# NCKempke/PIPS-IPMpp

Hardware: AMD Instinct MI355X
Metric: KKT factor+solve per IPM iter/sec, N-block arrowhead LP (higher is better)
Workload: dtype f64; 1 GPU; 64 blocks x 10000 vars (5000 eq rows, rho=0.001), Schur dim 2000, 64 blocks/GPU [BASELINE configs[1]]; deterministic=False, family=random, root=dense LDL^T, sparse_head=multifrontal (k_front), solves_per_unit=4, collective=none, nnzL_per_gpu=649118456

## Files before the change

### include/pips_hip.h

```cpp
#ifndef PIPS_HIP_H
#define PIPS_HIP_H
#include <stddef.h>
#include <stdint.h>

#ifdef __cplusplus
extern "C" {
#endif

const char* pips_hip_last_error(void);
long long pips_hip_host_wait_count(void);
int pips_hip_host_wait_sites(char* buf, int cap);
int pips_hip_device_count(void);

int pips_hip_ldl_create(void** handle, int n, const int* krow, const int* jcol, int device, int flags);
int pips_hip_ldl_set_inertia_hint(void* handle, int n_primal);
int pips_hip_ldl_set_pivot_rule(void* handle, double thr_rel, double repl_rel);
int pips_hip_ldl_set_refinement(void* handle, int max_steps, double tol);
int pips_hip_ldl_set_refinement_backward_error(void* handle, int max_steps, double tol);
int pips_hip_ldl_set_deterministic(void* handle, int on);
int pips_hip_ldl_analyze(void* handle);
int pips_hip_ldl_factor(void* handle, const double* vals_host);
int pips_hip_ldl_solve(void* handle, int nrhs, double* rhs_inout_host, int ld);
int pips_hip_ldl_inertia(void* handle, int* pos, int* neg, int* zero);
int pips_hip_ldl_set_border(void* handle, int S, const int* Bt_rowptr, const int* Bt_colidx);
int pips_hip_ldl_factor_schur(void* handle, const double* K_vals_host, const double* Bt_vals_host, double* SC_host, int ldSC);
int pips_hip_ldl_solve_dev(void* handle, int nrhs, double* rhs_inout_dev, long long ld);
int pips_hip_ldl_solve_sparse(void* handle, int nrhs, double* rhs_inout_host, int ld, const int* col_sparsity);
int pips_hip_ldl_factor_schur_batch(void* const* handles, int n, const double* const* K_vals_host, const double* const* Bt_vals_host,
                                    double* SC_host, int ldSC);
int pips_hip_ldl_solve_batch(void* const* handles, int n, double* const* rhs_inout_host);
int pips_hip_ldl_solve_batch_dev(void* const* handles, int n, double* x_dev);
int pips_hip_ldl_inertia_batch(void* const* handles, int n, int* pos, int* neg, int* zero);
int pips_hip_ldl_info(void* handle, int64_t* what, int n_what);
int pips_hip_ldl_get_perm(void* handle, int* perm);
void pips_hip_ldl_destroy(void* handle);

int pips_hip_dense_ldl_create(void** handle, int n, int n_primal, int device);
int pips_hip_dense_ldl_set_pivoting(void* handle, int mode);
int pips_root_plan_build(int ntc, int workers, int qmin, int urgent, int chain_slots, int* out, long long cap, long long* n_tasks,
                         long long* n_chain_tasks, double* makespan_us);
int pips_hip_dense_ldl_set_distributed(void* handle, void* comm, int rank, int n_ranks);
int pips_hip_dense_ldl_factor(void* handle, const double* A_host, int lda);
int pips_hip_dense_ldl_factor_dev(void* handle, const double* A_dev, int lda);
int pips_hip_dense_ldl_solve(void* handle, int nrhs, double* rhs_inout_host, int ld);
int pips_hip_dense_ldl_solve_dev(void* handle, double* rhs_inout_dev);
int pips_hip_dense_ldl_inertia(void* handle, int* pos, int* neg, int* zero);
void pips_hip_dense_ldl_destroy(void* handle);

int pips_hip_batch_create(void** handle, int n_blocks, int S, int device, void* stream);
int pips_hip_batch_set_block(void* handle, int b, int n, int n_primal, const int* K_rowptr, const int* K_colidx,
                             const int* Bt_rowptr, const int* Bt_colidx, const double* Bt_val);
int pips_hip_batch_set_options(void* handle, int force_n_head, int refine_steps, double thr_rel, double repl_rel);
int pips_hip_batch_set_schur_mode(void* handle, int mode);
int pips_hip_batch_get_schur_mode(void* handle, int* mode);
int pips_hip_batch_set_deterministic(void* handle, int on);
int pips_hip_batch_add_regularization(void* handle, double primal, double dual);
int pips_hip_batch_set_refinement(void* handle, int max_steps, double tol);
int pips_hip_batch_set_refinement_backward_error(void* handle, int max_steps, double tol);
double pips_hip_batch_last_refinement_measure(void* handle);
int pips_hip_batch_last_refinement_steps(void* handle);
int pips_hip_batch_analyze(void* handle, int n_threads);
int pips_hip_batch_set_values(void* handle, int b, const double* K_val_host);
int pips_hip_batch_set_diagonals_dev(void* handle, const double* diag_dev);
// ... 169 lines not shown
```

### pips-ipmpp_amd/csrc/engine.hip

```cpp
#include <hip/hip_runtime.h>

#include <algorithm>
#include <cstdlib>
#include <cstring>
#include <map>
#include <memory>
#include <mutex>
#include <thread>
#include <vector>

#include "common.h"
#include "kernels.hip.h"
#include "rootkernel.hip.h"
#include "tailkernel.hip.h"
#include "pips_hip.h"

namespace pips {

static thread_local std::string g_last_error;
void set_last_error(const std::string& msg) { g_last_error = msg; }
std::atomic<long long> g_host_waits{0};
struct WaitSite { std::atomic<const char*> file{nullptr}; std::atomic<int> line{0}; std::atomic<long long> n{0}; };
static WaitSite g_wait_sites[128];
void note_host_wait(const char* file, int line) {
// ... 28 lines not shown
   HIP_TRY(hipMalloc((void**)dptr, bytes));
   if (!h.empty()) HIP_TRY(hipMemcpy(*dptr, h.data(), h.size() * sizeof(T), hipMemcpyHostToDevice));
   return PIPS_OK;
}

static int env_int(const char* name, int dflt) {
   const char* v = getenv(name);
   return v ? atoi(v) : dflt;
}

static inline int grid_for(long long n, int block, int cap = 4096) {
   long long g = (n + block - 1) / block;
   if (g < 1) g = 1;
   if (g > cap) g = cap;
   return (int)g;
}

struct TaskList { long long off = 0; int cnt = 0; };

struct TailPlan {
   int ntc_max = 0;
   std::vector<TaskList> upd, upd_diag, diag, trsm, fwd, bwd, trail, trail_next;
   TaskList schur;
   TileTask* d_tasks = nullptr;
   std::vector<TileTask> h_tasks;

   int build(const std::vector<BlkDesc>& blks, int panel = 0, bool lookahead = false, bool split_diag = false,
             const std::vector<const std::vector<int>*>* first = nullptr, bool diag_ahead = false, int pair2 = 1) {
      std::vector<TileTask> all;
      ntc_max = 0;
      for (auto& b : blks) ntc_max = std::max(ntc_max, b.ntc);
      upd.assign(ntc_max, {});
      upd_diag.assign(ntc_max, {});
      diag.assign(ntc_max, {});
      trsm.assign(ntc_max, {});
      fwd.assign(ntc_max, {});
      bwd.assign(ntc_max, {});
      trail.assign(ntc_max, {});
      trail_next.assign(ntc_max, {});
      const int nblk = (int)blks.size();
      auto begin = [&](TaskList& l) { l.off = (long long)all.size(); };
      auto end = [&](TaskList& l) { l.cnt = (int)((long long)all.size() - l.off); };
      for (int j = 0; j < ntc_max; ++j) {
         const int p0 = panel > 0 ? j / panel * panel : 0;
         auto fst = [&](int b, int t) { return first ? (*(*first)[b])[t] : 0; };
         begin(upd_diag[j]);
         if (j > p0 && split_diag)
            for (int b = 0; b < nblk; ++b)
               if (blks[b].ntc > j) {
                  const int k0 = std::max(p0, fst(b, j));
                  if (k0 < j) all.push_back({b, j, j, (diag_ahead ? std::max(k0, j - 1) : k0) | (j << 16)});
               }
         end(upd_diag[j]);
         begin(upd[j]);
         const int P = (pair2 > 1 && panel == 0 && split_diag && diag_ahead) ? pair2 : 1;
         const int g = j / P * P, q = j - g;
         if (j > p0 && split_diag && diag_ahead)
            for (int b = 0; b < nblk; ++b)
               if (blks[b].ntc > j + 1) {
                  const int k0 = std::max(p0, fst(b, j + 1)), lo = q > 0 ? std::max(k0, g) : k0;
                  if (lo < j) all.push_back({b, j + 1, j + 1, lo | (j << 16)});
               }
         if (P > 1 && q == 0 && j > p0)
            for (int b = 0; b < nblk; ++b)
               for (int d = j + 2; d <= j + P && d < blks[b].ntc; ++d) {
                  const int k0 = std::max(p0, fst(b, d));
                  if (k0 < j) all.push_back({b, d, d, k0 | (j << 16)});
               }
         if (j > p0)
            for (int b = 0; b < nblk; ++b)
               if (blks[b].ntc > j)
                  for (int ti = split_diag ? j + 1 : j; ti < blks[b].ntr; ++ti) {
                     if (j >= fst(b, ti)) {
                        const int k0 = std::max({p0, fst(b, ti), fst(b, j)}), lo = q > 0 ? std::max(k0, g) : k0;
                        if (lo < j) all.push_back({b, ti, j, lo | (j << 16)});
                     }
                     if (P > 1 && q == 0)
                        for (int c = j + 1; c < j + P && c < blks[b].ntc && c < ti; ++c)
                           if (c >= fst(b, ti)) {
                              const int k0 = std::max({p0, fst(b, ti), fst(b, c)});
                              if (k0 < j) all.push_back({b, ti, c, k0 | (j << 16)});
                           }
                  }
         end(upd[j]);
         begin(diag[j]);
         for (int b = 0; b < nblk; ++b)
            if (blks[b].ntc > j) all.push_back({b, j, j, 0});
         end(diag[j]);
         begin(trsm[j]);
         for (int b = 0; b < nblk; ++b)
            if (blks[b].ntc > j)
               for (int ti = j + 1; ti < blks[b].ntr; ++ti)
                  if (j >= fst(b, ti)) all.push_back({b, ti, j, 0});
         end(trsm[j]);
         begin(fwd[j]);
         for (int b = 0; b < nblk; ++b)
            if (blks[b].ntc > j)
               for (int ti = j; ti < blks[b].ntc; ++ti)
                  if (ti == j || (j >= 1 && j - 1 >= fst(b, ti))) all.push_back({b, ti, j, 0});
         end(fwd[j]);
         begin(bwd[j]);
         for (int b = 0; b < nblk; ++b)
            if (blks[b].ntc > j)
               for (int tj = 0; tj <= j; ++tj)
                  if (tj == j || (j + 1 < blks[b].ntc && tj >= fst(b, j + 1))) all.push_back({b, tj, j, 0});
         end(bwd[j]);
         if (panel > 0 && (j + 1) % panel == 0) {
            begin(trail_next[j]);
            if (lookahead)
               for (int b = 0; b < nblk; ++b)
                  if (j + 1 < blks[b].ntc)
                     for (int ti = j + 1; ti < blks[b].ntr; ++ti) all.push_back({b, ti, j + 1, p0 | ((j + 1) << 16)});
            end(trail_next[j]);
            begin(trail[j]);
            for (int b = 0; b < nblk; ++b)
               for (int tj = j + (lookahead ? 2 : 1); tj < blks[b].ntc; ++tj)
                  for (int ti = tj; ti < blks[b].ntr; ++ti) all.push_back({b, ti, tj, p0 | ((j + 1) << 16)});
            end(trail[j]);
         }
      }
      begin(schur);
      for (int b = 0; b < nblk; ++b)
         if (blks[b].ntc > 0 && blks[b].nb > 0) {
            const int nt = blks[b].nb_pad / TILE;
            for (int ti = 0; ti < nt; ++ti)
               for (int tj = 0; tj <= ti; ++tj) all.push_back({b, ti, tj, 0});
         }
      end(schur);
      h_tasks = all;
      return dev_upload(&d_tasks, all, nullptr);
   }
   void release() {
      if (d_tasks) (void)hipFree(d_tasks);
      d_tasks = nullptr;
   }
};

struct SweepRt {
   TileTask* d_tasks = nullptr;
   int n_tasks = 0;
   int* d_ints = nullptr;
   long long n_flags = 0;
   long long* d_flag_off = nullptr;
   int* d_tfirst = nullptr;
   long long* d_tfirst_off = nullptr;
   int epoch = 0;
   bool enabled = false;
   long long poll_limit = SWEEP_POLL_LIMIT;
   int take_error(const char* who) {
      if (!d_ints) return PIPS_OK;
      int w = 0;
      HIP_TRY(hipMemcpy(&w, d_ints + 2 * SWEEP_NRHS_MAX, sizeof(int), hipMemcpyDeviceToHost));
      if (!w) return PIPS_OK;
// ... 197 lines not shown
   double* d_uarena = nullptr;
   const std::vector<TaskList>* sc_groups = nullptr;
   const TileTask* d_sc_tasks = nullptr;
   const std::vector<hipEvent_t>* ev_sc = nullptr;
   int* d_ctr_pool = nullptr;
   int* ctr_cursor = nullptr;
   const std::vector<TaskList>* det_rounds = nullptr;
   const TileTask* d_det_tasks = nullptr;
   double* d_gbuf = nullptr;
   long long gstride = 0;
   const int* d_blk_group = nullptr;
   int n_groups = 0, first_slot = 0;
   long long sc_len = 0;
   bool det_defer_reduce = false;
   bool det_reduce_later = false;
   SweepRt* sweep = nullptr;
   bool bunch_kaufman = false;
   int *d_pert_cnt = nullptr, *d_pert_list = nullptr;
   const double* bk_orig = nullptr;
   int bk_orig_ld = 0, bk_orig_rowmajor = 0;
   const int* d_bk_perm = nullptr;
   int bk_isolate = 0;
   const TailSingle* single = nullptr;
};
constexpr int GEMM_CTR_SLOTS = 4096;
constexpr int GEMM_BAL_MIN_TASKS = 1024;

static void reduce_det_groups(const TailCtx& c, double* SC, int ldSC) {
   const int S_ = ldSC;
   if (c.det_defer_reduce) {
   } else if (c.d_sctab)
      hipLaunchKernelGGL(k_reduce_groups, dim3((unsigned)std::max(1LL, std::min(1024LL, (c.sc_len + 255) / 256)), 1), dim3(256), 0, c.stream, SC, 0, (int)c.sc_len,
                         c.d_gbuf, c.gstride, c.n_groups, c.first_slot);
   else
      hipLaunchKernelGGL(k_reduce_groups, dim3(std::max(1, std::min(64, (S_ + 255) / 256)), S_), dim3(256), 0, c.stream, SC, ldSC, S_, c.d_gbuf,
                         c.gstride, c.n_groups, c.first_slot);
}

static int tail_factor(const TailCtx& c, double* SC, int ldSC) {
   const TailPlan& p = *c.plan;
   auto gemm_diag_tiles = [&](const TaskList& l, hipStream_t st) {
      hipLaunchKernelGGL(k_tile_gemm<4>, dim3((l.cnt + 7) / 8 * 8), dim3(512), 0, st, p.d_tasks + l.off, l.cnt, c.d_blks, c.d_arena,
                         c.d_dtail, c.d_winv, c.d_bmap, (double*)nullptr, 0, (const int*)nullptr, c.d_uarena);
   };
   auto gemm0 = [&](const TaskList& l, hipStream_t st) {
      if (!c.is_root && c.d_ctr_pool && l.cnt >= GEMM_BAL_MIN_TASKS && *c.ctr_cursor < GEMM_CTR_SLOTS) {
         int* ctr = c.d_ctr_pool + 8 * (*c.ctr_cursor)++;
         const int wgs = ((l.cnt + 7) / 8 * 8) / 8 * 9;
         hipLaunchKernelGGL(k_tile_gemm_bal<0>, dim3((wgs + 7) / 8 * 8), dim3(512), 0, st, p.d_tasks + l.off, l.cnt, c.d_blks, c.d_arena, c.d_dtail,
                            c.d_winv, c.d_bmap, (double*)nullptr, 0, (const int*)nullptr, c.d_uarena, ctr);
         return;
      }
      if (c.is_root)
         hipLaunchKernelGGL(k_tile_gemm<3>, dim3((l.cnt + 7) / 8 * 8), dim3(512), 0, st, p.d_tasks + l.off, l.cnt, c.d_blks, c.d_arena,
                            c.d_dtail, c.d_winv, c.d_bmap, (double*)nullptr, 0, (const int*)nullptr, c.d_uarena);
      else
         hipLaunchKernelGGL(k_tile_gemm<0>, dim3((l.cnt + 7) / 8 * 8), dim3(512), 0, st, p.d_tasks + l.off, l.cnt, c.d_blks, c.d_arena,
                            c.d_dtail, c.d_winv, c.d_bmap, (double*)nullptr, 0, (const int*)nullptr, c.d_uarena);
   };
   bool side_busy = false;
   int side_from = 0;
   auto main_writes = [&](int col) -> int {
      if (side_busy && col >= side_from) {
         HIP_TRY(hipStreamWaitEvent(c.stream, c.ev_rest, 0));
         side_busy = false;
      }
      return PIPS_OK;
   };
   int rc;
   if (c.single && c.single->n_tasks > 0) {
      const TailSingle& ts = *c.single;
      if (c.timer) c.timer->begin(c.stream, 2);
      HIP_TRY(hipMemcpyAsync(ts.d_flags, ts.d_flags_init, (size_t)ts.n_flags * sizeof(int), hipMemcpyDeviceToDevice, c.stream));
      HIP_TRY(hipMemsetAsync(ts.d_ctl, 0, 9 * sizeof(int), c.stream));
      TailLdlArgs ta = ts.args;
      ta.n_tasks = ts.n_tasks;
      const char* trace_file = getenv("PIPS_HIP_TAIL_TRACE");
      long long* d_trace = nullptr;
      const size_t n_trace = (size_t)3 * ts.n_tasks + 32 * (size_t)(p.ntc_max + 1);
      if (trace_file) {
         HIP_TRY(hipMalloc((void**)&d_trace, n_trace * sizeof(long long)));
         HIP_TRY(hipMemsetAsync(d_trace, 0, n_trace * sizeof(long long), c.stream));
         ta.trace = d_trace;
      }
      hipLaunchKernelGGL(k_tail_ldl, dim3(ts.n_blocks <= 2 ? 256 : 512), dim3(512), 0, c.stream, ta);
      if (c.timer) c.timer->end(c.stream);
      if (trace_file) {
         std::vector<long long> h(n_trace);
         std::vector<TileTask> ht((size_t)ts.n_tasks);
         HIP_TRY(hipStreamSynchronize(c.stream));
         HIP_TRY(hipMemcpy(h.data(), d_trace, h.size() * sizeof(long long), hipMemcpyDeviceToHost));
         HIP_TRY(hipMemcpy(ht.data(), ts.d_tasks, ht.size() * sizeof(TileTask), hipMemcpyDeviceToHost));
// ... 31 lines not shown
         gemm0(p.upd[j], c.stream);
         if (c.timer) c.timer->end(c.stream);
      }
      if (ahead) {
         HIP_TRY(hipStreamWaitEvent(c.stream, c.ev_rest, 0));
      } else {
         if (c.timer) c.timer->begin(c.stream, 3);
         if (c.bunch_kaufman)
            hipLaunchKernelGGL(k_tile_diag_bk, dim3(p.diag[j].cnt), dim3(256), 0, c.stream, p.d_tasks + p.diag[j].off, c.d_blks, c.d_arena, c.d_dtail,
                               c.d_winv, c.d_inertia, c.d_pert_cnt, c.d_pert_list, c.bk_orig, c.bk_orig_ld, c.bk_orig_rowmajor, c.d_bk_perm, c.bk_isolate);
         else
         hipLaunchKernelGGL(k_tile_diag, dim3(p.diag[j].cnt), dim3(256), 0, c.stream, p.d_tasks + p.diag[j].off,
                            c.d_blks, c.d_arena, c.d_dtail, c.d_winv, c.d_psign, c.d_psign_off, c.d_inertia, c.d_pref);
         if (c.timer) c.timer->end(c.stream);
      }
      if (p.trsm[j].cnt > 0) {
         if (c.timer) c.timer->begin(c.stream, 4);
         hipLaunchKernelGGL(k_tile_gemm<1>, dim3((p.trsm[j].cnt + 7) / 8 * 8), dim3(512), 0, c.stream, p.d_tasks + p.trsm[j].off, p.trsm[j].cnt,
                            c.d_blks, c.d_arena, c.d_dtail, c.d_winv, c.d_bmap, (double*)nullptr, 0, (const int*)nullptr, c.d_uarena);
         if (c.timer) c.timer->end(c.stream);
         if (c.bunch_kaufman && c.is_root && c.d_pert_cnt)
            hipLaunchKernelGGL(k_bk_growth, dim3(TILE), dim3(256), 0, c.stream, c.d_blks, c.d_arena, j, 1e8, c.d_pert_cnt, c.d_pert_list);
      }
      if (p.trail_next[j].cnt > 0 || p.trail[j].cnt > 0) {
         if ((rc = main_writes(j + 1))) return rc;
         const bool split = c.side && p.trail[j].cnt > 0;
         if (split) {
            HIP_TRY(hipEventRecord(c.ev_panel, c.stream));
            HIP_TRY(hipStreamWaitEvent(c.side, c.ev_panel, 0));
            gemm0(p.trail[j], c.side);
            HIP_TRY(hipEventRecord(c.ev_rest, c.side));
            side_busy = true;
            side_from = j + 2;
         }
         if (c.timer) c.timer->begin(c.stream, 2);
         if (p.trail_next[j].cnt > 0) gemm0(p.trail_next[j], c.stream);
         if (!split && p.trail[j].cnt > 0) gemm0(p.trail[j], c.stream);
         if (c.timer) c.timer->end(c.stream);
      }
   }
   if ((rc = main_writes(1 << 30))) return rc;
   if (SC && c.det_rounds) {
      if (c.timer) c.timer->begin(c.stream, 5);
      for (const TaskList& l : *c.det_rounds)
         if (l.cnt > 0)
            hipLaunchKernelGGL(k_tile_gemm<2>, dim3((l.cnt + 7) / 8 * 8), dim3(512), 0, c.stream, c.d_det_tasks + l.off, l.cnt, c.d_blks, c.d_arena,
                               c.d_dtail, c.d_winv, c.d_bmap, SC, ldSC, c.d_sctab, c.d_uarena, c.d_gbuf, c.gstride, c.d_blk_group);
      if (!c.det_reduce_later) reduce_det_groups(c, SC, ldSC);
      if (c.timer) c.timer->end(c.stream);
   } else if (SC && c.sc_groups && !c.d_sctab) {
      if (c.timer) c.timer->begin(c.stream, 5);
      for (size_t g = 0; g < c.sc_groups->size(); ++g) {
         const TaskList& l = (*c.sc_groups)[g];
         if (l.cnt > 0)
            hipLaunchKernelGGL(k_tile_gemm<2>, dim3((l.cnt + 7) / 8 * 8), dim3(512), 0, c.stream, c.d_sc_tasks + l.off, l.cnt, c.d_blks, c.d_arena,
                               c.d_dtail, c.d_winv, c.d_bmap, SC, ldSC, c.d_sctab, c.d_uarena);
         HIP_TRY(hipEventRecord((*c.ev_sc)[g], c.stream));
      }
      if (c.timer) c.timer->end(c.stream);
   } else if (SC && p.schur.cnt > 0 && c.d_ctr_pool && !c.d_sctab && *c.ctr_cursor < GEMM_CTR_SLOTS) {
      if (c.timer) c.timer->begin(c.stream, 5);
      const int wgs = ((p.schur.cnt + 7) / 8 * 8) / 8 * 9;
      hipLaunchKernelGGL(k_tile_gemm_bal<2>, dim3((wgs + 7) / 8 * 8), dim3(512), 0, c.stream, p.d_tasks + p.schur.off, p.schur.cnt, c.d_blks,
                         c.d_arena, c.d_dtail, c.d_winv, c.d_bmap, SC, ldSC, c.d_sctab, c.d_uarena, c.d_ctr_pool + 8 * (*c.ctr_cursor)++);
// ... 151 lines not shown
   long long *d_kdst = nullptr, *d_bdst = nullptr, *d_kdiag = nullptr, *d_kptr = nullptr, *d_psign_off = nullptr,
             *d_perm_off = nullptr, *d_rowbase = nullptr, *d_bt_xoff = nullptr;
   SnDesc* d_sns = nullptr;
   BlkDesc* d_blks = nullptr;
   int *d_lf_rows = nullptr, *d_lf_ptr = nullptr, *d_lf_src = nullptr, *d_lf_pos = nullptr;
   double* d_lf_val = nullptr;
   long long lf_rows = 0, lf_entries = 0;
   LeafDesc* d_leafdesc = nullptr;
   int* d_lb_list = nullptr;
   int n_lb = 0, nb_pad_max = 0;
   int head_wcap = HEAD_WMAX;
   int *d_rowidx = nullptr, *d_upd = nullptr, *d_sncol = nullptr, *d_bmap = nullptr, *d_perm = nullptr, *d_inertia = nullptr, *d_nprimal = nullptr;
   int *d_br_rowptr = nullptr, *d_br_sc = nullptr, *d_br_src = nullptr;
   int *d_krowptr = nullptr, *d_kcolidx = nullptr, *d_bt_rowptr = nullptr, *d_bt_colidx = nullptr, *d_bt_rowsc = nullptr;
   signed char* d_psign = nullptr;
   std::vector<int> h_inertia;
   std::vector<double> h_amax;

   ~Engine() {
      release();
      if (side) (void)hipStreamDestroy(side);
      if (ev_diag_in) (void)hipEventDestroy(ev_diag_in);
      if (ev_diag_out) (void)hipEventDestroy(ev_diag_out);
   }
   void release() {
      if (d_uarena) (void)hipFree(d_uarena);
      d_uarena = nullptr;
      for (auto ev : ev_sc) (void)hipEventDestroy(ev);
      ev_sc.clear(); sc_groups.clear(); sc_row_begin.clear();
      if (d_sc_tasks) (void)hipFree(d_sc_tasks);
      d_sc_tasks = nullptr;
      for (void* q : {(void*)d_lf_rows, (void*)d_lf_ptr, (void*)d_lf_src, (void*)d_lf_pos, (void*)d_lf_val})
         if (q) (void)hipFree(q);
      d_lf_rows = d_lf_ptr = d_lf_src = d_lf_pos = nullptr; d_lf_val = nullptr;
      for (void* q : {(void*)d_br_rowptr, (void*)d_br_sc, (void*)d_br_src})
         if (q) (void)hipFree(q);
      d_br_rowptr = d_br_sc = d_br_src = nullptr;
      if (d_leafdesc) (void)hipFree(d_leafdesc);
      d_leafdesc = nullptr;
      lf_rows = 0; lf_entries = 0;
      if (d_mfU) (void)hipFree(d_mfU);
      if (d_mfLV) (void)hipFree(d_mfLV);
      for (void* q : {(void*)d_bb_batches, (void*)d_bb_meta, (void*)d_bb_off, (void*)d_bb_pos, (void*)d_bb_round_blk, (void*)d_bb_out})
         if (q) (void)hipFree(q);
      d_bb_out = nullptr;
      d_bb_batches = nullptr; d_bb_meta = nullptr; d_bb_off = nullptr; d_bb_pos = nullptr; d_bb_round_blk = nullptr; n_bb = 0; bb_doubles = 0;
// ... 42 lines not shown
      h_mmeasure = nullptr;
      mx_cap = 0;
      hostx_cap = hostpack_cap = 0;
      d_kdst = d_bdst = d_kdiag = d_kptr = d_psign_off = d_perm_off = d_rowbase = d_bt_xoff = nullptr;
      d_sns = nullptr; d_blks = nullptr;
      d_nprimal = nullptr;
      d_spine = d_spine_off = d_schur_cols = d_schur_slot = d_sctab = nullptr;
      for (void* q : {(void*)d_kb_rec, (void*)d_kb_off, (void*)d_kb_list, (void*)d_kb_tail}) if (q) (void)hipFree(q);
      d_kb_rec = nullptr; d_kb_off = nullptr; d_kb_list = nullptr; d_kb_tail = nullptr; n_kb_tail = 0; kb_level_off.clear(); kb_level_pairs.clear(); kb_level_lds.clear();
      d_frowptr = d_fcol = d_fsrc = nullptr; d_flong = nullptr;
      d_rowidx = d_upd = d_sncol = d_bmap = d_perm = d_inertia = d_krowptr = d_kcolidx = d_bt_rowptr = d_bt_colidx = d_bt_rowsc = nullptr;
      d_psign = nullptr;
      plan.release();
      sweep.release();
      tsingle.release();
   }

   SweepRt sweep;
   TailSingle tsingle;
   bool tail_single = false;
   long long tail_scratch = 0;
   hipStream_t side = nullptr;
   hipEvent_t ev_diag_in = nullptr, ev_diag_out = nullptr;
   struct GatherList {
      long long n_targets = 0, n_slots = 0;
      long long *d_tgt = nullptr, *d_off = nullptr, *d_slots = nullptr;
      void release() {
         for (void* p : {(void*)d_tgt, (void*)d_off, (void*)d_slots})
            if (p) (void)hipFree(p);
         d_tgt = d_off = d_slots = nullptr;
         n_targets = n_slots = 0;
      }
   };
   struct SlotEntry { long long target, slot; };
   bool deterministic = false;
   bool head_slots = false;
   bool slot_solves = false;
   static constexpr long long HEAD_SLOTS_MAX = 400LL * 1000 * 1000;
   long long slots_total = 0, vslots_total = 0;
   double *d_slot_val = nullptr, *d_vslot_val = nullptr;
   int last_multi_path = 0;
   double* d_mvslot = nullptr;
   std::vector<GatherList> g_levels, gv_levels;
   GatherList g_tail, g_sc, gv_tail;
   std::vector<SlotEntry> sc_e_keep;
   std::vector<int> sc_blk_keep;
// ... 178 lines not shown
            int q = (int)(std::upper_bound(sc_row_begin.begin(), sc_row_begin.end(), first) - sc_row_begin.begin()) - 1;
            q = std::max(0, std::min(q, n_panels - 1));
            for (int tj = 0; tj <= ti; ++tj) g[q].push_back({b, ti, tj, 0});
         }
      }
      std::vector<TileTask> all;
      for (int q = 0; q < n_panels; ++q) {
         TaskList l;
         l.off = (long long)all.size(); l.cnt = (int)g[q].size();
         all.insert(all.end(), g[q].begin(), g[q].end());
         sc_groups.push_back(l);
         hipEvent_t ev;
         HIP_TRY(hipEventCreateWithFlags(&ev, hipEventDisableTiming));
         ev_sc.push_back(ev);
      }
      if (all.empty()) all.push_back({-1, 0, 0, 0});
      return dev_upload(&d_sc_tasks, all, stream);
   }
   TailCtx ctx() {
      TailCtx c{d_blks, &plan, d_arena, d_dtail, d_winv, d_psign, d_psign_off, d_bmap, d_inertia, stream,
                timer.on ? &timer : nullptr, d_pref, side, ev_diag_in, ev_diag_out, false, d_sctab, d_uarena};
      if (!sc_groups.empty()) { c.sc_groups = &sc_groups; c.d_sc_tasks = d_sc_tasks; c.ev_sc = &ev_sc; }
      c.d_ctr_pool = d_gemm_ctr; c.ctr_cursor = &gemm_ctr_cursor;
      if (deterministic && d_gbuf) {
         c.det_rounds = &det_rounds; c.d_det_tasks = d_det_tasks; c.d_gbuf = d_gbuf; c.gstride = det_gstride(); c.sc_len = sc_len; c.d_blk_group = d_blk_group;
         c.n_groups = det_n_groups; c.first_slot = det_first_slot;
         c.det_defer_reduce = det_global && defer_group_reduce;
      }
      c.sweep = &sweep;
      if (tail_single) {
         tsingle.args.blks = d_blks; tsingle.args.arena = d_arena; tsingle.args.uarena = d_uarena; tsingle.args.winv = d_winv; tsingle.args.dtail = d_dtail;
         tsingle.args.pref = d_pref; tsingle.args.psign = d_psign; tsingle.args.psign_off = d_psign_off; tsingle.args.inertia = d_inertia;
         c.single = &tsingle;
      }
      return c;
   }

   int analyze_host(int n_threads, bool with_border = true) {
      sym.assign(nblk, BlockSym());
      std::vector<int> rc(nblk, 0);
      std::vector<std::string> msgs(nblk);
      n_threads = std::max(1, std::min(n_threads, nblk));
      auto work = [&](int t) {
         for (int b = t; b < nblk; b += n_threads) {
            CsrPattern K{in[b].n, in[b].n, in[b].krow.data(), in[b].kcol.data()};
            CsrPattern B{0, in[b].n, nullptr, nullptr};
// ... 572 lines not shown
      if ((rc = dev_upload(&d_bt_rowsc, h_bt_rowsc, stream))) return rc;
      if (bt_rows_total > 0 && nnzB_total > 0 && nnzB_total < (1LL << 31)) {
         std::vector<int> rp((size_t)n_total + 1, 0);
         for (long long r = 0; r < bt_rows_total; ++r)
            for (int p = h_bt_rowptr[r]; p < h_bt_rowptr[r + 1]; ++p) ++rp[h_bt_xoff[r] + h_bt_colidx[p] + 1];
         for (long long i = 0; i < n_total; ++i) rp[i + 1] += rp[i];
         std::vector<int> sc((size_t)nnzB_total), src((size_t)nnzB_total), fill(rp.begin(), rp.end() - 1);
         for (long long r = 0; r < bt_rows_total; ++r)
            for (int p = h_bt_rowptr[r]; p < h_bt_rowptr[r + 1]; ++p) {
               const int q = fill[h_bt_xoff[r] + h_bt_colidx[p]]++;
               sc[q] = h_bt_rowsc[r]; src[q] = p;
            }
         if ((rc = dev_upload(&d_br_rowptr, rp, stream)) || (rc = dev_upload(&d_br_sc, sc, stream)) || (rc = dev_upload(&d_br_src, src, stream)))
            return rc;
      }
      {
         std::vector<int> np(nblk);
         for (int b = 0; b < nblk; ++b) np[b] = in[b].n_primal;
         if ((rc = dev_upload(&d_nprimal, np, stream))) return rc;
      }
      std::vector<const std::vector<int>*> firsts(nblk);
      for (int b = 0; b < nblk; ++b) firsts[b] = &sym[b].tile_first;
      const int pair2 = 4;
      if ((rc = plan.build(h_blks, 0, false, true, &firsts, true, pair2))) return rc;
      if ((rc = sweep.build(h_blks, &firsts))) return rc;
      if (tail_single) {
         if ((rc = tsingle.build(plan, h_blks, stream))) return rc;
         tsingle.args.poll_limit = env_int("PIPS_HIP_ROOT_POLL_LIMIT", 400000) > 0 ? (long long)env_int("PIPS_HIP_ROOT_POLL_LIMIT", 400000) * 50 : 0;
         tsingle.args.diag_blocked = env_int("PIPS_HIP_ROOT_DIAG_BARRIERS", 0) ? 0 : 1;
      }
      {
         double fwd_entries = 0.0, border_entries = 0.0;
         for (int b = 0; b < nblk; ++b) {
            const BlockSym& sb = sym[b];
            fwd_entries += 0.5 * (double)sb.m_pad * sb.m_pad;
            border_entries += (double)sb.nb_pad * sb.m_pad;
            for (const HeadSupernode& sn : sb.sn) {
               const int nbord = sn.r - sn.rb;
               fwd_entries += (double)sn.w * (sn.r - nbord) + 0.5 * sn.w * sn.w;
               border_entries += (double)sn.w * nbord;
            }
         }
         border_backward_ok = schur_mode_eff == 1 && nnzB_total > 0 && (sweep.enabled || plan.ntc_max == 0) && !deterministic && border_entries <= 3.0 * fwd_entries;
         if (const char* bb = getenv("PIPS_HIP_BORDER_BACKWARD"))
            border_backward_ok = atoi(bb) != 0 && schur_mode_eff == 1 && nnzB_total > 0 && sweep.enabled && !deterministic;
         const bool aug_paths = schur_mode_eff == 1 && nnzB_total > 0 && (sweep.enabled || plan.ntc_max == 0) && spine_total == 0 &&
                                (deterministic || !head_slots);
         aug_sweeps_ok = aug_paths && border_entries <= 3.0 * fwd_entries;
         if (const char* as = getenv("PIPS_HIP_AUG_SWEEPS")) aug_sweeps_ok = atoi(as) != 0 && aug_paths;
      }
      if (!side) {
         int prio_lo = 0, prio_hi = 0;
         HIP_TRY(hipDeviceGetStreamPriorityRange(&prio_lo, &prio_hi));
         HIP_TRY(hipStreamCreateWithPriority(&side, hipStreamNonBlocking, prio_hi));
         HIP_TRY(hipEventCreateWithFlags(&ev_diag_in, hipEventDisableTiming));
         HIP_TRY(hipEventCreateWithFlags(&ev_diag_out, hipEventDisableTiming));
      }
      h_inertia.assign(3 * nblk, 0);
      slots_total = slots_acc; vslots_total = vslots_acc;
      h_sns_keep = h_sns;
      analyzed = true;
      ++analysis_gen;
      factored = false;
      head_slots = false;
      const bool want_slots = deterministic;
      if (want_slots && slots_total + vslots_total <= HEAD_SLOTS_MAX) {
         if ((rc = build_deterministic(n_threads))) return rc;
         head_slots = true;
      } else if (deterministic)
         PIPS_FAIL(PIPS_ERR_STATE, "deterministic mode: %lld head contributions exceed the slot budget of %lld", slots_total + vslots_total, HEAD_SLOTS_MAX);
      if (deterministic && (rc = set_det_groups(0, 1))) return rc;
      return PIPS_OK;
   }

   std::vector<SnDesc> h_sns_keep;
   ScatterCtx sx_atomic() const { return ScatterCtx{0, nullptr, nullptr, nullptr, nullptr}; }
   void launch_head_level(const LevelRange& L, double* SC, int ldSC, const ScatterCtx& sx) {
      if (L.simple_cnt > 0)
         hipLaunchKernelGGL(k_head_factor_simple, dim3((L.simple_cnt + 255) / 256), dim3(256), 0, stream, d_sns, L.simple_begin,
// ... 3391 lines not shown
   }
   std::vector<int> hv(hubs, hubs + n_hubs), pv, cc;
   if (!hub_dissected_order(n, ap, ai, hv, min_size, pv, cc)) PIPS_FAIL(PIPS_ERR_STATE, "pips_symbolic_probe_hubs: no separators");
   AnalyzeOptions opt;
   apply_tuning(opt);
   opt.user_perm = pv.data();
   opt.user_colcount = cc.data();
   {
      int cut = 0;
      while (cut < n - n_hubs && cc[cut] <= ROOT_ND_MAX_COLCOUNT) ++cut;
      opt.force_n_head = cut;
   }
   CsrPattern K{n, n, krow, jcol};
   CsrPattern B{0, n, nullptr, nullptr};
   std::vector<BlockSym> sym(1);
   int rc = analyze_block(K, B, n_primal, opt, sym[0]);
   if (rc) return rc;
   if (what) sym_info(sym, what, n_what);
   if (perm) std::copy(sym[0].perm.begin(), sym[0].perm.end(), perm);
   if (colcount) std::copy(sym[0].colcount.begin(), sym[0].colcount.end(), colcount);
   return PIPS_OK;
}

}
```

### pips-ipmpp_amd/csrc/kernels.hip.h

```cpp
#pragma once
#include <hip/hip_runtime.h>
#include <stdint.h>

namespace pips {

constexpr int TILE = 128;
constexpr int KB = 16;
constexpr int LDS_PAD = 16;
constexpr int LDSW = TILE + LDS_PAD;

struct SnDesc {
   long long panel;
   long long rows;
   long long upd;
   int w, r, c0, blk;
   int n_useg, rb;
   int ld, pad_;
   long long slot;
   long long vslot;
   long long U;
   long long mf;
   long long bb;
};

// ... 1472 lines not shown
                                                         const int* __restrict__ sctab, double* __restrict__ uarena,
                                                         int* __restrict__ ctr) {
   __shared__ GemmShared sh;
   __shared__ int s_tix;
   if (threadIdx.x == 0) {
      const int per = (n_tasks + 7) >> 3;
      const int xcc = (int)(__builtin_amdgcn_s_getreg((3 << 11) | 20 ) & 7);
      int got = -1;
      for (int d = 0; d < 8 && got < 0; ++d) {
         const int x = (xcc + d) & 7;
         if (__hip_atomic_load(ctr + x, __ATOMIC_RELAXED, __HIP_MEMORY_SCOPE_AGENT) >= per) continue;
         const int t = __hip_atomic_fetch_add(ctr + x, 1, __ATOMIC_RELAXED, __HIP_MEMORY_SCOPE_AGENT);
         const int tix = x * per + t;
         if (t < per && tix < n_tasks) got = tix;
      }
      s_tix = got;
   }
   __syncthreads();
   const int tix = s_tix;
   if (tix < 0) return;
   tile_gemm_body<MODE>(tix, sh, tasks, n_tasks, blks, arena, dtail, winv, bmap, SC, ldSC, sctab, uarena);
}

__global__ void k_reduce_groups(double* __restrict__ SC, int ld, int S, const double* __restrict__ gbuf, long long gstride, int n_groups,
                                int first_slot) {
   const int c = blockIdx.y;
   for (int r = c + blockIdx.x * blockDim.x + threadIdx.x; r < S; r += gridDim.x * blockDim.x) {
      const long long off = r + (long long)c * ld;
      double p[8];
#pragma unroll
      for (int g = 0; g < 8; ++g) {
         const int lg = g - first_slot;
         p[g] = (lg >= 0 && lg < n_groups) ? gbuf[lg * gstride + off] : 0.0;
      }
      SC[off] += ((p[0] + p[1]) + (p[2] + p[3])) + ((p[4] + p[5]) + (p[6] + p[7]));
   }
}



struct DiagShared {
   double colk[2][TILE];
   double xrow[2][TILE];
   double dk[TILE];
   double prs[TILE];
   int sgn[TILE];
// ... 1720 lines not shown
```

### pips-ipmpp_amd/python/capi.py

```python
import ctypes as C
import sys
import os

import numpy as np

try:
    import torch
except Exception:
    torch = None

_HERE = os.path.dirname(os.path.abspath(__file__))
LIB_PATH = os.environ.get("PIPS_HIP_LIBRARY") or os.path.join(os.path.dirname(_HERE), "libpipship.so")


class PipsHipError(RuntimeError):
    pass


def _load():
    if not os.path.exists(LIB_PATH):
        raise PipsHipError(
            f"{LIB_PATH} is missing: build it with `python -c 'import __graft_entry__ as g; g.build()'` "
            "(hipcc --offload-arch=gfx950). The MI355X backend has no CPU fallback.")
    return C.CDLL(LIB_PATH, mode=C.RTLD_GLOBAL)


lib = _load()

_i32p = np.ctypeslib.ndpointer(dtype=np.int32, flags="C_CONTIGUOUS")
_f64p = np.ctypeslib.ndpointer(dtype=np.float64, flags="C_CONTIGUOUS")
_i64p = np.ctypeslib.ndpointer(dtype=np.int64, flags="C_CONTIGUOUS")
_vp = C.c_void_p

lib.pips_hip_last_error.restype = C.c_char_p
lib.pips_hip_device_count.restype = C.c_int
lib.pips_hip_host_wait_count.restype = C.c_longlong

SYMBOLS = [
    "pips_hip_last_error", "pips_hip_device_count",
    "pips_hip_ldl_create", "pips_hip_ldl_set_inertia_hint", "pips_hip_ldl_set_pivot_rule", "pips_hip_ldl_set_refinement", "pips_hip_ldl_set_refinement_backward_error", "pips_hip_ldl_set_deterministic",
    "pips_hip_ldl_analyze", "pips_hip_ldl_factor", "pips_hip_ldl_solve", "pips_hip_ldl_inertia", "pips_hip_ldl_info",
    "pips_hip_ldl_get_perm", "pips_hip_ldl_set_border", "pips_hip_ldl_factor_schur", "pips_hip_ldl_destroy",
    "pips_hip_ldl_solve_dev", "pips_hip_ldl_solve_sparse", "pips_hip_ldl_factor_schur_batch", "pips_hip_ldl_solve_batch", "pips_hip_ldl_solve_batch_dev",
    "pips_hip_ldl_inertia_batch",
    "pips_hip_dense_ldl_create", "pips_hip_dense_ldl_factor", "pips_hip_dense_ldl_factor_dev", "pips_hip_dense_ldl_solve",
    "pips_hip_dense_ldl_solve_dev", "pips_hip_dense_ldl_inertia", "pips_hip_dense_ldl_set_pivoting", "pips_hip_dense_ldl_set_distributed", "pips_hip_dense_ldl_destroy", "pips_root_plan_build", "pips_hip_host_wait_count", "pips_hip_host_wait_sites",
    "pips_hip_batch_create", "pips_hip_batch_set_block", "pips_hip_batch_set_options", "pips_hip_batch_set_schur_mode", "pips_hip_batch_set_deterministic", "pips_hip_batch_get_schur_mode", "pips_hip_batch_add_regularization", "pips_hip_batch_set_refinement",
    "pips_hip_batch_last_refinement_steps", "pips_hip_batch_set_refinement_backward_error",
    "pips_hip_batch_last_refinement_measure", "pips_hip_batch_analyze",
    "pips_hip_batch_set_values", "pips_hip_batch_set_diagonals_dev", "pips_hip_batch_set_diagonals", "pips_hip_batch_factor",
    "pips_hip_batch_solve_dev", "pips_hip_batch_solve", "pips_hip_batch_border_tmult_dev", "pips_hip_batch_border_mult_dev",
    "pips_hip_batch_inertia", "pips_hip_batch_info", "pips_hip_batch_sync", "pips_hip_batch_set_timing",
    "pips_hip_batch_get_timing", "pips_hip_batch_destroy",
    "pips_hip_kkt_create", "pips_hip_kkt_create_sparse", "pips_hip_kkt_get_schur_sparse", "pips_hip_kkt_sparse_root_info", "pips_hip_kkt_factorize", "pips_hip_kkt_set_root_regularization", "pips_hip_kkt_solve_compressed", "pips_hip_kkt_get_schur",
    "pips_hip_kkt_set_root_inequalities", "pips_hip_kkt_set_zdiag0_dev",
    "pips_hip_kkt_root_inertia", "pips_hip_kkt_get_timing", "pips_hip_kkt_last_ltsolve_from_factor", "pips_hip_kkt_last_solve_path", "pips_hip_kkt_set_solve_check", "pips_hip_kkt_solve_check_counts", "pips_hip_kkt_set_solve_graph", "pips_hip_kkt_set_root_stream", "pips_hip_kkt_solve_graph_stats", "pips_hip_kkt_set_root_pivoting", "pips_hip_kkt_destroy",
    "pips_hip_malloc", "pips_hip_free", "pips_hip_memcpy_h2d", "pips_hip_memcpy_d2h", "pips_hip_memset",
    "pips_hip_comm_unique_id", "pips_hip_comm_create", "pips_hip_comm_create_external", "pips_hip_comm_set_external_rsag", "pips_hip_comm_set_external_broadcast", "pips_hip_broadcast", "pips_hip_comm_has_broadcast", "pips_hip_allreduce_sum_rsag", "pips_hip_all_gather", "pips_hip_comm_size", "pips_hip_allreduce_sum", "pips_hip_comm_destroy",
    "pips_hip_vec_axpy", "pips_hip_vec_axpby", "pips_hip_vec_scale", "pips_hip_vec_copy", "pips_hip_vec_set",
    "pips_hip_vec_add_const", "pips_hip_vec_mul", "pips_hip_vec_div", "pips_hip_vec_add_product", "pips_hip_vec_add_quotient",
    "pips_hip_vec_divide_some", "pips_hip_vec_select_nonzeros", "pips_hip_vec_safe_invert", "pips_hip_vec_gondzio_projection", "pips_hip_vec_dot",
    "pips_hip_vec_one_norm", "pips_hip_vec_inf_norm", "pips_hip_vec_min", "pips_hip_vec_sumsq_scaled", "pips_hip_vec_stepbound",
    "pips_hip_vec_find_blocking", "pips_hip_vec_weighted_stepbounds", "pips_hip_vec_dot_shifted", "pips_ipm_create", "pips_ipm_create_rank", "pips_ipm_create_general", "pips_ipm_get_dims", "pips_ipm_get_iterate", "pips_ipm_get_stats2", "pips_ipm_get_schur_mode", "pips_ipm_mult", "pips_ipm_outer_solve", "pips_ipm_solve", "pips_ipm_set_gondzio", "pips_ipm_set_option", "pips_ipm_set_free_variables", "pips_ipm_get_solution", "pips_ipm_get_trace", "pips_ipm_get_stats", "pips_ipm_destroy",
    "pips_gdx_read_block", "pips_gdx_block_counts", "pips_gdx_block_vector", "pips_gdx_block_matrix", "pips_gdx_block_destroy",
    "pips_gen_row_nnz", "pips_gen_block", "pips_gen_root", "pips_gen_diagonal", "pips_kkt_leaf_assemble",
    "pips_border_assemble", "pips_symbolic_probe", "pips_symbolic_probe_hubs", "pips_map_children_to_ranks",
]


# ... 968 lines not shown
```

Baseline: 8.239 64-block work units/s (1 factorize + 4 solveCompressed).

## Defer border-row tile updates into strip kernels on a low-priority side stream

Removes border rows (ti >= ntc) from the per-column update and trsm task lists. They are processed instead in column strips of width W (default 4) by a new k_border_strip kernel. That kernel runs update, update and trsm sequentially per column inside one block, on a low-priority stream that overlaps with the main diagonal/panel chain. The goal is to shorten the critical path of the tail factorization by taking the bulk border work off the per-column launches. The cost is extra event synchronization, possible contention between streams, and fine-grained ordering inside the strip kernel that relies on threadfence and syncthreads. A host-only planning export is also added for testing.

```diff
diff --git a/include/pips_hip.h b/include/pips_hip.h
--- a/include/pips_hip.h
+++ b/include/pips_hip.h
@@ -39,6 +39,8 @@
 int pips_hip_dense_ldl_set_pivoting(void* handle, int mode);
 int pips_root_plan_build(int ntc, int workers, int qmin, int urgent, int chain_slots, int* out, long long cap, long long* n_tasks,
                          long long* n_chain_tasks, double* makespan_us);
+int pips_tail_plan_tasks(int nblk, const int* ntc, const int* ntr, const int* first, int pair2, int strips, int* out, long long cap,
+                         long long* n_rows);
 int pips_hip_dense_ldl_set_distributed(void* handle, void* comm, int rank, int n_ranks);
 int pips_hip_dense_ldl_factor(void* handle, const double* A_host, int lda);
 int pips_hip_dense_ldl_factor_dev(void* handle, const double* A_dev, int lda);
diff --git a/pips-ipmpp_amd/csrc/engine.hip b/pips-ipmpp_amd/csrc/engine.hip
--- a/pips-ipmpp_amd/csrc/engine.hip
+++ b/pips-ipmpp_amd/csrc/engine.hip
@@ -74,12 +74,16 @@
    int ntc_max = 0;
    std::vector<TaskList> upd, upd_diag, diag, trsm, fwd, bwd, trail, trail_next;
    TaskList schur;
+   int strip_w = 0;
+   std::vector<TaskList> strip;
    TileTask* d_tasks = nullptr;
    std::vector<TileTask> h_tasks;
+   bool host_only = false;
 
    int build(const std::vector<BlkDesc>& blks, int panel = 0, bool lookahead = false, bool split_diag = false,
-             const std::vector<const std::vector<int>*>* first = nullptr, bool diag_ahead = false, int pair2 = 1) {
+             const std::vector<const std::vector<int>*>* first = nullptr, bool diag_ahead = false, int pair2 = 1, int strips = 0) {
       std::vector<TileTask> all;
+      strip_w = panel == 0 ? std::max(strips, 0) : 0;
       ntc_max = 0;
       for (auto& b : blks) ntc_max = std::max(ntc_max, b.ntc);
       upd.assign(ntc_max, {});
@@ -93,9 +97,11 @@
       const int nblk = (int)blks.size();
       auto begin = [&](TaskList& l) { l.off = (long long)all.size(); };
       auto end = [&](TaskList& l) { l.cnt = (int)((long long)all.size() - l.off); };
+      auto fst = [&](int b, int t) { return first ? (*(*first)[b])[t] : 0; };
+      const int P = (pair2 > 1 && panel == 0 && split_diag && diag_ahead) ? pair2 : 1;
+      auto rows_end = [&](int b) { return strip_w > 0 ? blks[b].ntc : blks[b].ntr; };
       for (int j = 0; j < ntc_max; ++j) {
          const int p0 = panel > 0 ? j / panel * panel : 0;
-         auto fst = [&](int b, int t) { return first ? (*(*first)[b])[t] : 0; };
          begin(upd_diag[j]);
          if (j > p0 && split_diag)
             for (int b = 0; b < nblk; ++b)
@@ -105,7 +111,6 @@
                }
          end(upd_diag[j]);
          begin(upd[j]);
-         const int P = (pair2 > 1 && panel == 0 && split_diag && diag_ahead) ? pair2 : 1;
          const int g = j / P * P, q = j - g;
          if (j > p0 && split_diag && diag_ahead)
             for (int b = 0; b < nblk; ++b)
@@ -122,7 +127,7 @@
          if (j > p0)
             for (int b = 0; b < nblk; ++b)
                if (blks[b].ntc > j)
-                  for (int ti = split_diag ? j + 1 : j; ti < blks[b].ntr; ++ti) {
+                  for (int ti = split_diag ? j + 1 : j; ti < rows_end(b); ++ti) {
                      if (j >= fst(b, ti)) {
                         const int k0 = std::max({p0, fst(b, ti), fst(b, j)}), lo = q > 0 ? std::max(k0, g) : k0;
                         if (lo < j) all.push_back({b, ti, j, lo | (j << 16)});
@@ -142,7 +147,7 @@
          begin(trsm[j]);
          for (int b = 0; b < nblk; ++b)
             if (blks[b].ntc > j)
-               for (int ti = j + 1; ti < blks[b].ntr; ++ti)
+               for (int ti = j + 1; ti < rows_end(b); ++ti)
                   if (j >= fst(b, ti)) all.push_back({b, ti, j, 0});
          end(trsm[j]);
          begin(fwd[j]);
@@ -171,6 +176,28 @@
             end(trail[j]);
          }
       }
+      strip.assign(strip_w > 0 ? (ntc_max + strip_w - 1) / strip_w : 0, {});
+      for (size_t sp = 0; sp < strip.size(); ++sp) {
+         begin(strip[sp]);
+         const int c0 = (int)sp * strip_w;
+         for (int b = 0; b < nblk; ++b)
+            if (blks[b].ntc > c0)
+               for (int ti = blks[b].ntc; ti < blks[b].ntr; ++ti)
+                  for (int c = c0; c < c0 + strip_w; ++c) {
+                     TileTask u1{-1, 0, 0, 0}, u2{-1, 0, 0, 0}, tr{-1, 0, 0, 0};
+                     if (c < blks[b].ntc && c >= fst(b, ti)) {
+                        const int k0 = std::max(fst(b, ti), fst(b, c)), g = c / P * P, lo = std::max(k0, g);
+                        if (g > 0 && k0 < g) u1 = {b, ti, c, k0 | (g << 16)};
+                        if (lo < c) u2 = {b, ti, c, lo | (c << 16)};
+                        tr = {b, ti, c, 0};
+                     }
+                     all.push_back(u1);
+                     all.push_back(u2);
+                     all.push_back(tr);
+                  }
+         end(strip[sp]);
+         strip[sp].cnt /= 3 * strip_w;
+      }
       begin(schur);
       for (int b = 0; b < nblk; ++b)
          if (blks[b].ntc > 0 && blks[b].nb > 0) {
@@ -180,7 +207,7 @@
          }
       end(schur);
       h_tasks = all;
-      return dev_upload(&d_tasks, all, nullptr);
+      return host_only ? PIPS_OK : dev_upload(&d_tasks, all, nullptr);
    }
    void release() {
       if (d_tasks) (void)hipFree(d_tasks);
@@ -424,6 +451,9 @@
    const int* d_bk_perm = nullptr;
    int bk_isolate = 0;
    const TailSingle* single = nullptr;
+   hipStream_t strips = nullptr;
+   hipEvent_t ev_strip_in = nullptr;
+   hipEvent_t ev_strip_out = nullptr;
 };
 constexpr int GEMM_CTR_SLOTS = 4096;
 constexpr int GEMM_BAL_MIN_TASKS = 1024;
@@ -470,6 +500,7 @@
       return PIPS_OK;
    };
    int rc;
+   bool strips_queued = false;
    if (c.single && c.single->n_tasks > 0) {
       const TailSingle& ts = *c.single;
       if (c.timer) c.timer->begin(c.stream, 2);
@@ -547,6 +578,21 @@
          if (c.bunch_kaufman && c.is_root && c.d_pert_cnt)
             hipLaunchKernelGGL(k_bk_growth, dim3(TILE), dim3(256), 0, c.stream, c.d_blks, c.d_arena, j, 1e8, c.d_pert_cnt, c.d_pert_list);
       }
+      if (p.strip_w > 0 && ((j + 1) % p.strip_w == 0 || j + 1 == p.ntc_max)) {
+         const TaskList& l = p.strip[j / p.strip_w];
+         const hipStream_t st = c.strips ? c.strips : c.stream;
+         if (l.cnt > 0) {
+            if (st != c.stream) {
+               HIP_TRY(hipEventRecord(c.ev_strip_in, c.stream));
+               HIP_TRY(hipStreamWaitEvent(st, c.ev_strip_in, 0));
+               strips_queued = true;
+            }
+            if (c.timer) c.timer->begin(st, 2);
+            hipLaunchKernelGGL(k_border_strip, dim3((l.cnt + 7) / 8 * 8), dim3(512), 0, st, p.d_tasks + l.off, l.cnt, p.strip_w, c.d_blks,
+                               c.d_arena, c.d_dtail, c.d_winv, c.d_uarena);
+            if (c.timer) c.timer->end(st);
+         }
+      }
       if (p.trail_next[j].cnt > 0 || p.trail[j].cnt > 0) {
          if ((rc = main_writes(j + 1))) return rc;
          const bool split = c.side && p.trail[j].cnt > 0;
@@ -565,6 +611,10 @@
       }
    }
    if ((rc = main_writes(1 << 30))) return rc;
+   if (strips_queued) {
+      HIP_TRY(hipEventRecord(c.ev_strip_out, c.strips));
+      HIP_TRY(hipStreamWaitEvent(c.stream, c.ev_strip_out, 0));
+   }
    if (SC && c.det_rounds) {
       if (c.timer) c.timer->begin(c.stream, 5);
       for (const TaskList& l : *c.det_rounds)
@@ -762,6 +812,9 @@
       if (side) (void)hipStreamDestroy(side);
       if (ev_diag_in) (void)hipEventDestroy(ev_diag_in);
       if (ev_diag_out) (void)hipEventDestroy(ev_diag_out);
+      if (strip_stream) (void)hipStreamDestroy(strip_stream);
+      if (ev_strip_in) (void)hipEventDestroy(ev_strip_in);
+      if (ev_strip_out) (void)hipEventDestroy(ev_strip_out);
    }
    void release() {
       if (d_uarena) (void)hipFree(d_uarena);
@@ -850,6 +903,8 @@
    long long tail_scratch = 0;
    hipStream_t side = nullptr;
    hipEvent_t ev_diag_in = nullptr, ev_diag_out = nullptr;
+   hipStream_t strip_stream = nullptr;
+   hipEvent_t ev_strip_in = nullptr, ev_strip_out = nullptr;
    struct GatherList {
       long long n_targets = 0, n_slots = 0;
       long long *d_tgt = nullptr, *d_off = nullptr, *d_slots = nullptr;
@@ -1074,6 +1129,7 @@
                 timer.on ? &timer : nullptr, d_pref, side, ev_diag_in, ev_diag_out, false, d_sctab, d_uarena};
       if (!sc_groups.empty()) { c.sc_groups = &sc_groups; c.d_sc_tasks = d_sc_tasks; c.ev_sc = &ev_sc; }
       c.d_ctr_pool = d_gemm_ctr; c.ctr_cursor = &gemm_ctr_cursor;
+      c.strips = strip_stream; c.ev_strip_in = ev_strip_in; c.ev_strip_out = ev_strip_out;
       if (deterministic && d_gbuf) {
          c.det_rounds = &det_rounds; c.d_det_tasks = d_det_tasks; c.d_gbuf = d_gbuf; c.gstride = det_gstride(); c.sc_len = sc_len; c.d_blk_group = d_blk_group;
          c.n_groups = det_n_groups; c.first_slot = det_first_slot;
@@ -1692,7 +1748,8 @@
       std::vector<const std::vector<int>*> firsts(nblk);
       for (int b = 0; b < nblk; ++b) firsts[b] = &sym[b].tile_first;
       const int pair2 = 4;
-      if ((rc = plan.build(h_blks, 0, false, true, &firsts, true, pair2))) return rc;
+      const int strips = tail_single ? 0 : std::max(0, env_int("PIPS_HIP_BORDER_STRIPS", 4));
+      if ((rc = plan.build(h_blks, 0, false, true, &firsts, true, pair2, strips))) return rc;
       if ((rc = sweep.build(h_blks, &firsts))) return rc;
       if (tail_single) {
          if ((rc = tsingle.build(plan, h_blks, stream))) return rc;
@@ -1725,6 +1782,13 @@
          HIP_TRY(hipStreamCreateWithPriority(&side, hipStreamNonBlocking, prio_hi));
          HIP_TRY(hipEventCreateWithFlags(&ev_diag_in, hipEventDisableTiming));
          HIP_TRY(hipEventCreateWithFlags(&ev_diag_out, hipEventDisableTiming));
+      }
+      if (!strip_stream && plan.strip_w > 0) {
+         int prio_lo = 0, prio_hi = 0;
+         HIP_TRY(hipDeviceGetStreamPriorityRange(&prio_lo, &prio_hi));
+         HIP_TRY(hipStreamCreateWithPriority(&strip_stream, hipStreamNonBlocking, prio_lo));
+         HIP_TRY(hipEventCreateWithFlags(&ev_strip_in, hipEventDisableTiming));
+         HIP_TRY(hipEventCreateWithFlags(&ev_strip_out, hipEventDisableTiming));
       }
       h_inertia.assign(3 * nblk, 0);
       slots_total = slots_acc; vslots_total = vslots_acc;
@@ -5162,4 +5226,46 @@
    return PIPS_OK;
 }
 
-}
+int pips_tail_plan_tasks(int nblk, const int* ntc, const int* ntr, const int* first, int pair2, int strips, int* out, long long cap,
+                         long long* n_rows) {
+   if (nblk < 0 || !ntc || !ntr || !n_rows) PIPS_FAIL(PIPS_ERR_ARG, "pips_tail_plan_tasks: bad arguments");
+   std::vector<BlkDesc> blks(nblk);
+   std::vector<std::vector<int>> fst(nblk);
+   std::vector<const std::vector<int>*> firsts(nblk);
+   long long at = 0;
+   for (int b = 0; b < nblk; ++b) {
+      std::memset(&blks[b], 0, sizeof(BlkDesc));
+      blks[b].ntc = ntc[b];
+      blks[b].ntr = ntr[b];
+      fst[b].assign(ntr[b], 0);
+      if (first) for (int t = 0; t < ntr[b]; ++t) fst[b][t] = first[at + t];
+      at += ntr[b];
+      firsts[b] = &fst[b];
+   }
+   TailPlan p;
+   p.host_only = true;
+   int rc = p.build(blks, 0, false, true, &firsts, true, pair2, strips);
+   if (rc) return rc;
+   std::vector<int> rows;
+   auto put = [&](const TaskList& l, int kind, int j) {
+      for (long long q = l.off; q < l.off + (kind == 4 ? 3LL * p.strip_w * l.cnt : l.cnt); ++q) {
+         const TileTask& t = p.h_tasks[q];
+         rows.insert(rows.end(), {kind, j, t.blk, t.ti, t.tj, t.pad});
+      }
+   };
+   for (int j = 0; j < p.ntc_max; ++j) {
+      put(p.upd_diag[j], 0, j);
+      put(p.diag[j], 1, j);
+      put(p.upd[j], 2, j);
+      put(p.trsm[j], 3, j);
+   }
+   for (size_t sp = 0; sp < p.strip.size(); ++sp) put(p.strip[sp], 4, (int)sp);
+   *n_rows = (long long)rows.size() / 6;
+   if (out) {
+      if (cap < (long long)rows.size()) PIPS_FAIL(PIPS_ERR_ARG, "pips_tail_plan_tasks: out holds %lld ints, %zu needed", cap, rows.size());
+      std::copy(rows.begin(), rows.end(), out);
+   }
+   return PIPS_OK;
+}
+
+}
diff --git a/pips-ipmpp_amd/csrc/kernels.hip.h b/pips-ipmpp_amd/csrc/kernels.hip.h
--- a/pips-ipmpp_amd/csrc/kernels.hip.h
+++ b/pips-ipmpp_amd/csrc/kernels.hip.h
@@ -1518,6 +1518,28 @@
    tile_gemm_body<MODE>(tix, sh, tasks, n_tasks, blks, arena, dtail, winv, bmap, SC, ldSC, sctab, uarena);
 }
 
+__global__ __launch_bounds__(512, 4) void k_border_strip(const TileTask* __restrict__ tasks, int n_strips, int W,
+                                                        const BlkDesc* __restrict__ blks, double* __restrict__ arena,
+                                                        const double* __restrict__ dtail, const double* __restrict__ winv,
+                                                        double* __restrict__ uarena) {
+   __shared__ GemmShared sh;
+   const int per = (n_strips + 7) >> 3;
+   const int s = (int)(blockIdx.x & 7) * per + (int)(blockIdx.x >> 3);
+   if (s >= n_strips) return;
+   const int base = 3 * W * s, n = 3 * W * n_strips;
+   for (int q = 0; q < W; ++q) {
+      tile_gemm_body<0>(base + 3 * q, sh, tasks, n, blks, arena, dtail, winv, nullptr, nullptr, 0, nullptr, uarena);
+      __threadfence();
+      __syncthreads();
+      tile_gemm_body<0>(base + 3 * q + 1, sh, tasks, n, blks, arena, dtail, winv, nullptr, nullptr, 0, nullptr, uarena);
+      __threadfence();
+      __syncthreads();
+      tile_gemm_body<1>(base + 3 * q + 2, sh, tasks, n, blks, arena, dtail, winv, nullptr, nullptr, 0, nullptr, uarena);
+      __threadfence();
+      __syncthreads();
+   }
+}
+
 __global__ void k_reduce_groups(double* __restrict__ SC, int ld, int S, const double* __restrict__ gbuf, long long gstride, int n_groups,
                                 int first_slot) {
    const int c = blockIdx.y;
diff --git a/pips-ipmpp_amd/python/capi.py b/pips-ipmpp_amd/python/capi.py
--- a/pips-ipmpp_amd/python/capi.py
+++ b/pips-ipmpp_amd/python/capi.py
@@ -44,7 +44,7 @@
     "pips_hip_ldl_solve_dev", "pips_hip_ldl_solve_sparse", "pips_hip_ldl_factor_schur_batch", "pips_hip_ldl_solve_batch", "pips_hip_ldl_solve_batch_dev",
     "pips_hip_ldl_inertia_batch",
     "pips_hip_dense_ldl_create", "pips_hip_dense_ldl_factor", "pips_hip_dense_ldl_factor_dev", "pips_hip_dense_ldl_solve",
-    "pips_hip_dense_ldl_solve_dev", "pips_hip_dense_ldl_inertia", "pips_hip_dense_ldl_set_pivoting", "pips_hip_dense_ldl_set_distributed", "pips_hip_dense_ldl_destroy", "pips_root_plan_build", "pips_hip_host_wait_count", "pips_hip_host_wait_sites",
+    "pips_hip_dense_ldl_solve_dev", "pips_hip_dense_ldl_inertia", "pips_hip_dense_ldl_set_pivoting", "pips_hip_dense_ldl_set_distributed", "pips_hip_dense_ldl_destroy", "pips_root_plan_build", "pips_tail_plan_tasks", "pips_hip_host_wait_count", "pips_hip_host_wait_sites",
     "pips_hip_batch_create", "pips_hip_batch_set_block", "pips_hip_batch_set_options", "pips_hip_batch_set_schur_mode", "pips_hip_batch_set_deterministic", "pips_hip_batch_get_schur_mode", "pips_hip_batch_add_regularization", "pips_hip_batch_set_refinement",
     "pips_hip_batch_last_refinement_steps", "pips_hip_batch_set_refinement_backward_error",
     "pips_hip_batch_last_refinement_measure", "pips_hip_batch_analyze",
```

Result: slower. 6.723 64-block work units/s (1 factorize + 4 solveCompressed) (median of 2 runs) (-18.4%).
